# ZeldaM1/PnP-VCVE

Measured on AMD Instinct MI355X. Metric: enhanced frames/sec (1280x720, 7-frame window), higher is better.
Workload: dtype f32; 1 GPU; 1 x 7x3x720x1280 clip per GPU per step (BASELINE configs[2] shape), full BAE+CAA forward, config HR_davis_LR_128x128 generator, seeded random weights; side info per SURVEY 8(d): partition class ~ U{0,1,2} per 8x8 block (one-hot/255, none on the I frame), quarter-pel block MVs, IBBBP cadence; vsr_x4_heads=False, hip_graphs=False, deform=vos, parallelism=clip-sharded replicas x1

## Files before the change

### pnp_vcve_amd/csrc/conv_wino.hip

```cpp
#include "conv_mfma.h"
#include <cstring>
#include <type_traits>

namespace {

template <int N>
using I = std::integral_constant<int, N>;
typedef unsigned u32x4 __attribute__((ext_vector_type(4)));

constexpr int HP = 18, NPX = HP * HP;
constexpr int SLAB_B = NPX * 64;
constexpr int RING_B = 4 * 16384;
constexpr int PV_B = RING_B + 4 * SLAB_B;
constexpr int BG_B = PV_B + 256 * 48;
constexpr int DUMP_B = BG_B + 256;
constexpr int WINO_LDS = DUMP_B + 1024;
constexpr unsigned OOBW = 0xFFFFFFF0u;

__device__ __forceinline__ f32x4 mfma16(float a, float b, f32x4 c) { return __builtin_amdgcn_mfma_f32_16x16x4f32(a, b, c, 0, 0, 0); }
__device__ __forceinline__ __amdgpu_buffer_rsrc_t rsrc_of(const void* p, unsigned bytes) {
    return __builtin_amdgcn_make_buffer_rsrc(const_cast<void*>(p), 0, __builtin_amdgcn_readfirstlane((int)bytes), 0x00020000);
}
__device__ __forceinline__ f32x4 bload4(__amdgpu_buffer_rsrc_t r, unsigned voff, unsigned soff) {
    return __builtin_bit_cast(f32x4, __builtin_amdgcn_raw_buffer_load_b128(r, (int)voff, (int)soff, 0));
// ... 80 lines not shown
    if (tile >= tend) return;

    const unsigned map_bytes = (unsigned)H * (unsigned)W * 256u;
    __amdgpu_buffer_rsrc_t r_src = rsrc_of(reinterpret_cast<const char*>(MS ? a.srcs[0] : a.src) - ((long)W + 1) * 256, OOBW);
    const __amdgpu_buffer_rsrc_t r_u = rsrc_of(MS ? a.ubase : a.U, MS ? OOBW : 16u * 16384u);
    const __amdgpu_buffer_rsrc_t r_urgb = rsrc_of(MS ? a.Urgb : a.U, 4u * 4096u);
    const __amdgpu_buffer_rsrc_t r_rgb = rsrc_of(reinterpret_cast<const char*>(MS ? a.rgb : a.src) - ((long)W + 1) * 16, OOBW);
    const __amdgpu_buffer_rsrc_t r_up = rsrc_of((PAR || FO) ? a.Upar : a.U, 4u * 12288u);
    const __amdgpu_buffer_rsrc_t r_out = rsrc_of(a.out, map_bytes);
    const __amdgpu_buffer_rsrc_t r_res = rsrc_of(RES ? a.residual : a.src, RES ? map_bytes : 0u);
    const __amdgpu_buffer_rsrc_t r_par = rsrc_of(a.par, PAR ? (unsigned)(3 * a.par_plane * 4) : 0u);

    const unsigned t16 = (unsigned)t * 16u;
    const int ty = 4 * (wave >> 1) + (m >> 2), tx = 4 * (wave & 1) + (m & 3);
    const unsigned dbase0 = RING_B + ((2 * ty) * HP + tx) * 64 + kq * 16, dbase1 = dbase0 + 2 * SLAB_B;
    auto lds4 = [&](unsigned byte) -> f32x4 { return *reinterpret_cast<const f32x4*>(smem + byte); };
    auto patch = [&](auto s_c, int r, int c) -> f32x4 {
        constexpr int S = decltype(s_c)::value;
        const unsigned off = (S & 1) * SLAB_B + (r * HP + (c & 1) * 9 + (c >> 1)) * 64;
        return lds4((S < 2 ? dbase0 : dbase1) + off);
    };

    const float act_lo = a.act == 0 ? 1.f : (a.act == 1 ? 0.f : 0.1f);
    if (t < 64) *reinterpret_cast<float*>(smem + BG_B + ((t & 15) * 4 + (t >> 4)) * 4) = (a.bias ? a.bias[t] : 0.f) * (a.gamma ? a.gamma[t] : 1.f);

    f32x4 acc[16][4];
    f32x4 V[16], d0[4], d1[4], d2[4], d3[4], bf[2][4], breg[4], hreg[3], tt[4];
    unsigned hoff[6];

    auto row_tf = [&](int i) {
        f32x4 tt[4];
#pragma unroll
        for (int c = 0; c < 4; ++c) tt[c] = i == 0 ? d0[c] - d2[c] : (i == 1 ? d1[c] + d2[c] : (i == 2 ? d2[c] - d1[c] : d1[c] - d3[c]));
        V[4 * i + 0] = tt[0] - tt[2];
        V[4 * i + 1] = tt[1] + tt[2];
        V[4 * i + 2] = tt[2] - tt[1];
        V[4 * i + 3] = tt[1] - tt[3];
    };
    auto halo_offsets = [&](int tq, int y0, int x0) {
#pragma unroll
        for (int i = 0; i < 6; ++i) {
            int e = tq + 256 * i;
            e = e < NPX * 4 ? e : NPX * 4 - 1;
            const int pl = e >> 2, quad = e & 3, ry = (pl * 3641) >> 16, col = pl - ry * HP;
            const int rx = col < 9 ? 2 * col : 2 * col - 17;
            const int gy = y0 - 1 + ry, gx = x0 - 1 + rx;
            const bool inb = (unsigned)gy < (unsigned)H && (unsigned)gx < (unsigned)W;
// ... 326 lines not shown
#pragma unroll
                            for (int c = 0; c < 4; ++c)
                                tt[c] = TR == 1 ? da[c] + db[c] : da[c] - db[c];
                        }
                        if (XF && g == 17) {
#pragma unroll
                            for (int c = 0; c < 4; ++c) {
                                V[4 * TR + c] = c == 0 ? tt[0] - tt[2] : (c == 1 ? tt[1] + tt[2] : (c == 2 ? tt[2] - tt[1] : tt[1] - tt[3]));
                                asm volatile("" : "+v"(V[4 * TR + c]));
                            }
                        }
                    } else {
                        if (g >= 20 && g < 28) {
                            const int c = (g - 20) & 3;
                            if (g < 24) da[c] = patch(SR{}, RA, c);
                            else db[c] = patch(SR{}, RB, c);
                        }
#pragma unroll
                        for (int c = 0; c < 4; ++c)
                            if (g == 36) tt[c] = TR == 1 ? add4(da[c], db[c]) : sub4(da[c], db[c]);
#pragma unroll
                        for (int c = 0; c < 4; ++c)
                            if (g == 36) V[4 * TR + c] = c == 0 ? sub4(tt[0], tt[2]) : (c == 1 ? add4(tt[1], tt[2]) : (c == 2 ? sub4(tt[2], tt[1]) : sub4(tt[1], tt[3])));
                    }
                    if constexpr (FO) {
                        if (PG == 0 && g >= 14 && g < 18) wjl[g - 14] = bload4(r_up, bl, fo_so + S * 12288 + (g - 14) * 1024);
                        if (PG == 1 && g >= 2 && g < 5) *reinterpret_cast<f32x4*>(smem + PV_B + (g - 2) * 4096 + tq16) = wjl[g - 2];
                        if (PG == 1 && g == 5) wj3 = wjl[3];
                    }
                    if constexpr (PAR || FO) {
                        if ((PG == 1 || PG == 2) && (g == 11 || g == 12 || g == 13 || g == 27 || g == 28 || g == 29)) {
                            wjt[(g & 15) - 11] = lds4(PV_B + ((g & 15) - 11) * 4096 + tq16);
                        }
                        if ((PG == 1 || PG == 2) && (g == 15 || g == 31)) {
                            {
                                const int pjn = (g + 1) >> 4;
                                const float cs = ((PG == 1) == (pjn == 1)) ? foldc : -foldc;
                                const f32x4 c4 = {cs, cs, cs, cs};
#pragma unroll
                                for (int n = 0; n < 3; ++n) bf[pjn & 1][n] = __builtin_elementwise_fma(c4, wjt[n], bf[pjn & 1][n]);
                                bf[pjn & 1][3] = __builtin_elementwise_fma(c4, wj3, bf[pjn & 1][3]);
                            }
                        }
                    }
                    if (PAR && g >= 52 && g < 52 + NRING) *reinterpret_cast<f32x4*>(smem + (NC & 3) * 16384 + (g - 52) * 4096 + tq16) = breg[g - 52];
                    if (!PAR && g == 63) {
// ... 97 lines not shown
                r_src = rsrc_of(reinterpret_cast<const char*>(a.srcs[last_seg ? 0 : ks + 1]) - ((long)W + 1) * 256, OOBW);
                ref_so = last_seg ? nso : (unsigned)(ty0 * W + tx0) * 256u;
                int tqs = tq;
                asm volatile("" : "+v"(tqs));
                halo_offsets(tqs, last_seg ? nty0 : ty0, last_seg ? ntx0 : tx0);
                step(I<0>{});
                step(I<1>{});
                step(I<2>{});
                step(I<3>{});
            }
        } else {
            step(I<0>{});
            step(I<1>{});
            step(I<2>{});
            step(I<3>{});
        }
        if (a.dbg) {
            dbg_b = __builtin_amdgcn_s_memtime();
            dbg_k += dbg_b - dbg_a;
        }

        const unsigned so = (unsigned)(ty0 * W + tx0) * 256u;
        const bool partial = ty0 + 16 > H || tx0 + 16 > W;
        lds_bar();
        const int tqp = (!has_next && qtile >= 0) ? ((qquad << 6) | (tq & 63)) : tq;
        pv_request(tqp, nty0, ntx0);
        fo_request(nty0, ntx0, (!has_next && qtile >= 0) ? qquad : -1);
        auto epilogue = [&](auto partial_c) {
            constexpr bool PARTIAL = decltype(partial_c)::value;
            int te = tq;
            asm volatile("" : "+v"(te));
            const int lq = te & 63, wq = te >> 6, kqq = lq >> 4, mq = lq & 15;
            char* tr = smem + 3 * 16384 + wq * 4096;
            const unsigned wbase = (unsigned)((2 * kqq) * 8 * 64 + mq * 4);
            const unsigned rbase = (unsigned)((lq >> 2) * 64 + (lq & 3) * 16);
            unsigned go[4];
#pragma unroll
            for (int j = 0; j < 4; ++j) {
                const int row = 8 * (wq >> 1) + 2 * j + (lq >> 5), col = 8 * (wq & 1) + ((lq >> 2) & 7);
                go[j] = (unsigned)(row * W + col) * 256u + (unsigned)(lq & 3) * 16u;
                if (PARTIAL) go[j] = (ty0 + row < H && tx0 + col < W) ? go[j] : OOBW;
            }
            f32x4 rs[4];
            if (RES) {
#pragma unroll
                for (int j = 0; j < 4; ++j) rs[j] = bload4(r_res, go[j], so);
            }
#pragma unroll
            for (int n = 0; n < 4; ++n) {
                f32x4 w0[4], w1[4];
#pragma unroll
                for (int i = 0; i < 4; ++i) {
                    w0[i] = acc[i * 4 + 0][n] + acc[i * 4 + 1][n] + acc[i * 4 + 2][n];
                    w1[i] = acc[i * 4 + 1][n] - acc[i * 4 + 2][n] - acc[i * 4 + 3][n];
                }
                f32x4 y[4];
                y[0] = w0[0] + w0[1] + w0[2];
                y[1] = w1[0] + w1[1] + w1[2];
                y[2] = w0[1] - w0[2] - w0[3];
                y[3] = w1[1] - w1[2] - w1[3];
#pragma unroll
                for (int q = 0; q < 4; ++q) {
#pragma unroll
                    for (int r = 0; r < 4; ++r) *reinterpret_cast<float*>(tr + wbase + ((q >> 1) * 8 + 2 * r + (q & 1)) * 64) = y[q][r];
                }
                f32x4 o[4];
#pragma unroll
                for (int j = 0; j < 4; ++j) o[j] = *reinterpret_cast<const f32x4*>(tr + rbase + j * 1024);
#pragma unroll
                for (int j = 0; j < 4; ++j) {
                    if constexpr (!RES) o[j] = __builtin_elementwise_max(o[j], act_lo * o[j]);
                    if (RES) {
                        o[j] += rs[j];
                        if (n < 3) rs[j] = bload4(r_res, go[j], so + (n + 1) * 64);
                    }
                    bstore4(r_out, go[j], so + n * 64, o[j]);
                }
            }
        };
        if (partial) epilogue(std::true_type{});
        else epilogue(std::false_type{});
        pv_finish(tqp);
        fo_finish();
        ++dbg_n;
        if (a.dbg) dbg_e += __builtin_amdgcn_s_memtime() - dbg_b;
        if (!has_next) break;
        tile = ntile;
        ty0 = nty0;
        tx0 = ntx0;
        if constexpr (SEAM) {
            f32x4 e0[4], e1[4], e2[4];
#pragma unroll
            for (int c = 0; c < 4; ++c) {
                e0[c] = patch(I<0>{}, 0, c);
                e1[c] = patch(I<0>{}, 1, c);
                e2[c] = patch(I<0>{}, 2, c);
            }
#pragma unroll
            for (int i = 0; i < 3; ++i) {
                f32x4 tr[4];
#pragma unroll
                for (int c = 0; c < 4; ++c) tr[c] = i == 0 ? e0[c] - e2[c] : (i == 1 ? e1[c] + e2[c] : e2[c] - e1[c]);
                V[4 * i + 0] = tr[0] - tr[2];
                V[4 * i + 1] = tr[1] + tr[2];
                V[4 * i + 2] = tr[2] - tr[1];
                V[4 * i + 3] = tr[1] - tr[3];
            }
        }
    }
    if constexpr (!PAR) wait_vm<0>();
    if constexpr (!MS) {
        const int qy0 = (qtile / tiles_x) * 16 + 8 * (qquad >> 1), qx0 = (qtile % tiles_x) * 16 + 8 * (qquad & 1);
        if (qtile >= 0 && qy0 < H && qx0 < W) {
            if (a.dbg) dbg_q0 = __builtin_amdgcn_s_memtime();
            const int tyq = m >> 2, txq = m & 3;
            const unsigned wq16 = (unsigned)lane * 16u + (unsigned)wave * 1024u;
            const unsigned qb0 = RING_B + ((2 * (4 * (qquad >> 1) + tyq)) * HP + 4 * (qquad & 1) + txq) * 64 + kq * 16, qb1 = qb0 + 2 * SLAB_B;
            f32x4 Bq[2][16], Bp[2][3];
#pragma unroll
            for (int p = 0; p < 16; ++p) Bq[0][p] = bload4(r_u, wq16, (unsigned)((p >> 2) * 16384 + (p & 3) * 4096));
            if constexpr (PAR) {
#pragma unroll
                for (int j = 0; j < 3; ++j) Bp[0][j] = bload4(r_up, wq16, (unsigned)(j * 4096));
            }
            f32x4 Bf[2];
            const int foq = FO ? __builtin_amdgcn_readfirstlane(fo_next) : -1;
            const unsigned foq_so = (unsigned)(foq > 0 ? foq : 0) * 4096u;
            if constexpr (FO) Bf[0] = bload4(r_up, wq16, foq_so);
            const unsigned qo = (unsigned)((qy0 + 2 * kq) * W + qx0) * 256u + (unsigned)(wave * 16 + m) * 4u;
            float resq[16];
            if constexpr (RES) {
#pragma unroll
                for (int q = 0; q < 4; ++q)
#pragma unroll
                    for (int r = 0; r < 4; ++r) {
                        const bool inq = qy0 + 2 * kq + (q >> 1) < H && qx0 + 2 * r + (q & 1) < W;
                        resq[q * 4 + r] = bload1(r_res, inq ? qo : OOBW, (unsigned)((q >> 1) * W + 2 * r + (q & 1)) * 256u);
                    }
            }
            const float bgq = *reinterpret_cast<const float*>(smem + BG_B + (m * 4 + wave) * 4);
            if constexpr (PAR) {
#pragma unroll
                for (int n = 0; n < 1; ++n) acc[0][0] = acc[3][0] = acc[12][0] = acc[15][0] = f32x4{0.f, 0.f, 0.f, 0.f};
            }
            lds_bar();
            if (a.dbg) dbg_q1 = __builtin_amdgcn_s_memtime();
            int needq = (PAR && a.par_flags) ? __builtin_amdgcn_readfirstlane(need_next) : 7;
            const int foldq = PAR ? __builtin_amdgcn_readfirstlane(fold_next) : -1;
            const float foldcq = PAR ? __builtin_bit_cast(float, __builtin_amdgcn_readfirstlane(__builtin_bit_cast(int, foldc_next)))
                                     : (FO ? __builtin_bit_cast(float, __builtin_amdgcn_readfirstlane(__builtin_bit_cast(int, foc_next))) : 0.f);
            if (foldq >= 0) needq = 0;
#pragma unroll
            for (int s4 = 0; s4 < 4; ++s4) {
                if (s4 < 3) {
#pragma unroll
                    for (int p = 0; p < 16; ++p) Bq[(s4 + 1) & 1][p] = bload4(r_u, wq16, (unsigned)(((s4 + 1) * 4 + (p >> 2)) * 16384 + (p & 3) * 4096));
                    if constexpr (PAR) {
#pragma unroll
                        for (int j = 0; j < 3; ++j) Bp[(s4 + 1) & 1][j] = bload4(r_up, wq16, (unsigned)((s4 + 1) * 12288 + j * 4096));
                    }
                    if constexpr (FO) Bf[(s4 + 1) & 1] = bload4(r_up, wq16, (unsigned)((s4 + 1) * 12288) + foq_so);
                }
                f32x4 dq[4][4], tq4[4];
// ... 147 lines not shown
    f32x4 hv[7];
    {
#pragma unroll
        for (int i = 0; i < 7; ++i) {
            const int e = t + 256 * i, pe = e >> 4, ry = pe / 10, rx = pe - ry * 10, gy = qy0 - 1 + ry, gx = qx0 - 1 + rx;
            hv[i] = f32x4{0.f, 0.f, 0.f, 0.f};
            if (e < 1600 && (unsigned)gy < (unsigned)H && (unsigned)gx < (unsigned)W)
                hv[i] = *reinterpret_cast<const f32x4*>(a.src + ((long)gy * W + gx) * 64 + (e & 15) * 4);
        }
        if constexpr (PAR) {
#pragma unroll
            for (int j = 0; j < 3; ++j)
#pragma unroll
                for (int q = 0; q < 4; ++q) {
                    const int gy = min(qy0 + 2 * tyq + (q >> 1), H - 1), gx = min(qx0 + 2 * txq + (q & 1), W - 1);
                    praw[j][q] = a.par[(long)j * a.par_plane + (long)gy * W + gx];
                }
        }
        if constexpr (FO) {
#pragma unroll
            for (int j = 0; j < 3; ++j) praw[j][0] = a.par[(long)j * a.par_plane + (long)qy0 * W + qx0];
        }
    }
    const unsigned wq16 = (unsigned)lane * 16u + (unsigned)wave * 1024u;
    constexpr int QA = 2, QB = QA + 1;
    f32x4 Bq[QB][16], Bp[QB][FO ? 1 : 3];
#pragma unroll
    for (int s0 = 0; s0 < QA; ++s0) {
#pragma unroll
        for (int p = 0; p < 16; ++p) Bq[s0][p] = bload4(r_u, wq16, (unsigned)((s0 * 4 + (p >> 2)) * 16384 + (p & 3) * 4096));
        if constexpr (PAR) {
#pragma unroll
            for (int j = 0; j < 3; ++j) Bp[s0][j] = bload4(r_up, wq16, (unsigned)(s0 * 12288 + j * 4096));
        }
    }
    int needq = 7, foldq = -1;
    float foldcq = 0.f;
    if constexpr (FO) {
        needq = 0;
#pragma unroll
        for (int j = 2; j >= 0; --j) {
            const float uv = __builtin_bit_cast(float, __builtin_amdgcn_readfirstlane(__builtin_bit_cast(int, praw[j][0])));
            if (uv != 0.f) {
                foldq = j;
                foldcq = 0.25f * uv;
            }
        }
// ... 182 lines not shown
#pragma unroll
        for (int i = 0; i < 7; ++i) {
            const int e = t + 256 * i, pe = e >> 4, ry = pe / 10, rx = pe - ry * 10, gy = qy0 - 1 + ry, gx = qx0 - 1 + rx;
            hv[i] = f32x4{0.f, 0.f, 0.f, 0.f};
            if (e < 1600 && (unsigned)gy < (unsigned)H && (unsigned)gx < (unsigned)W)
                hv[i] = *reinterpret_cast<const f32x4*>(src + ((long)gy * W + gx) * 64 + (e & 15) * 4);
        }
    };
    auto halo_store = [&](int buf) {
#pragma unroll
        for (int i = 0; i < 7; ++i) {
            const int e = t + 256 * i;
            if (e < 1600) *reinterpret_cast<f32x4*>(smem + buf * HB + (e >> 4) * QSTR + (e & 15) * 16) = hv[i];
        }
    };
    halo_request(a.srcs[0]);
    if (t < 100) {
        const int ry = t / 10, rx = t - ry * 10, gy = qy0 - 1 + ry, gx = qx0 - 1 + rx;
        f32x4 v = {0.f, 0.f, 0.f, 0.f};
        if ((unsigned)gy < (unsigned)H && (unsigned)gx < (unsigned)W) v = *reinterpret_cast<const f32x4*>(a.rgb + ((long)gy * W + gx) * 4);
        *reinterpret_cast<f32x4*>(smem + 2 * HB + t * 16) = v;
    }
    const int tyq = m >> 2, txq = m & 3;
    const unsigned wq16 = (unsigned)lane * 16u + (unsigned)wave * 1024u;
    f32x4 Bq[2][16], Br[16];
#pragma unroll
    for (int p = 0; p < 16; ++p) Br[p] = bload4(r_urgb, (unsigned)lane * 16u, (unsigned)((p >> 2) * 4096 + (p & 3) * 1024));
#pragma unroll
    for (int p = 0; p < 16; ++p) Bq[0][p] = bload4(r_u, wq16, a.u_off[0] + (unsigned)((p >> 2) * 16384 + (p & 3) * 4096));
    halo_store(0);
    const float bgq = a.bias ? a.bias[wave * 16 + m] : 0.f;
    f32x4 acc[16], V[16];
    lds_bar();
    {
        float dr[16], tr[16], Vr[16];
#pragma unroll
        for (int r = 0; r < 4; ++r)
#pragma unroll
            for (int c = 0; c < 4; ++c) dr[r * 4 + c] = *reinterpret_cast<const float*>(smem + 2 * HB + ((2 * tyq + r) * 10 + 2 * txq + c) * 16 + kq * 4);
#pragma unroll
        for (int c = 0; c < 4; ++c) {
            tr[0 * 4 + c] = dr[0 * 4 + c] - dr[2 * 4 + c];
            tr[1 * 4 + c] = dr[1 * 4 + c] + dr[2 * 4 + c];
            tr[2 * 4 + c] = dr[2 * 4 + c] - dr[1 * 4 + c];
            tr[3 * 4 + c] = dr[1 * 4 + c] - dr[3 * 4 + c];
        }
#pragma unroll
        for (int i = 0; i < 4; ++i) {
            Vr[i * 4 + 0] = tr[i * 4 + 0] - tr[i * 4 + 2];
            Vr[i * 4 + 1] = tr[i * 4 + 1] + tr[i * 4 + 2];
            Vr[i * 4 + 2] = tr[i * 4 + 2] - tr[i * 4 + 1];
            Vr[i * 4 + 3] = tr[i * 4 + 1] - tr[i * 4 + 3];
        }
#pragma unroll
        for (int p = 0; p < 16; ++p) {
            const f32x4 c0 = p == 5 ? f32x4{bgq, bgq, bgq, bgq} : f32x4{0.f, 0.f, 0.f, 0.f};
            const float bw = wave == 0 ? Br[p][0] : (wave == 1 ? Br[p][1] : (wave == 2 ? Br[p][2] : Br[p][3]));
            acc[p] = mfma16(Vr[p], bw, c0);
        }
    }
    for (int ks = 0; ks < a.nsrc; ++ks) {
        const bool more = ks + 1 < a.nsrc;
        const int buf = ks & 1;
        if (more) halo_request(a.srcs[ks + 1]);
#pragma unroll
        for (int s4 = 0; s4 < 4; ++s4) {
            if (s4 < 3) {
#pragma unroll
                for (int p = 0; p < 16; ++p)
                    Bq[(s4 + 1) & 1][p] = bload4(r_u, wq16, a.u_off[ks] + (unsigned)(((s4 + 1) * 4 + (p >> 2)) * 16384 + (p & 3) * 4096));
            } else if (more) {
#pragma unroll
                for (int p = 0; p < 16; ++p) Bq[0][p] = bload4(r_u, wq16, a.u_off[ks + 1] + (unsigned)((p >> 2) * 16384 + (p & 3) * 4096));
            }
            f32x4 dq[4][4], tq4[4];
#pragma unroll
            for (int r = 0; r < 4; ++r)
#pragma unroll
                for (int c = 0; c < 4; ++c)
                    dq[r][c] = *reinterpret_cast<const f32x4*>(smem + buf * HB + ((2 * tyq + r) * 10 + 2 * txq + c) * QSTR + (16 * s4 + 4 * kq) * 4);
#pragma unroll
// ... 34 lines not shown
    yq[2] = w0[1] - w0[2] - w0[3];
    yq[3] = w1[1] - w1[2] - w1[3];
    const unsigned qo = (unsigned)((qy0 + 2 * kq) * W + qx0) * 256u + (unsigned)(wave * 16 + m) * 4u;
#pragma unroll
    for (int q = 0; q < 4; ++q) {
        yq[q] = __builtin_elementwise_max(yq[q], act_lo * yq[q]);
#pragma unroll
        for (int r = 0; r < 4; ++r) {
            const bool inq = qy0 + 2 * kq + (q >> 1) < H && qx0 + 2 * r + (q & 1) < W;
            bstore1(r_out, inq ? qo : OOBW, (unsigned)((q >> 1) * W + 2 * r + (q & 1)) * 256u, yq[q][r]);
        }
    }
}
#endif
#ifndef WINO_MS_TU

struct WinoImgArgs {
    const float* src[16];
    float* dst[16];
    const float* gamma;
};
__global__ __launch_bounds__(256) void wino_image_kernel(const WinoImgArgs a) {
    const int idx = blockIdx.x * 256 + threadIdx.x;
    const int ci = ((idx >> 10) & 3) * 16 + ((idx >> 6) & 3) * 4 + (idx & 3), co = ((idx >> 8) & 3) * 16 + ((idx >> 2) & 15);
    const float* s = a.src[blockIdx.y];
    float* d = a.dst[blockIdx.y];
    double g[3][3];
#pragma unroll
    for (int tap = 0; tap < 9; ++tap)
        g[tap / 3][tap % 3] = s[tap * 4096 + (((ci >> 3) * 2 + (co >> 5)) * 64 + ((ci >> 2) & 1) * 32 + (co & 31)) * 4 + (ci & 3)];
    const double gm = a.gamma ? (double)a.gamma[co] : 1.0;
    double tmp[4][3];
#pragma unroll
    for (int x = 0; x < 3; ++x) {
        tmp[0][x] = g[0][x];
        tmp[1][x] = 0.5 * (g[0][x] + g[1][x] + g[2][x]);
        tmp[2][x] = 0.5 * (g[0][x] - g[1][x] + g[2][x]);
        tmp[3][x] = g[2][x];
    }
#pragma unroll
    for (int i = 0; i < 4; ++i) {
        const double u[4] = {tmp[i][0], 0.5 * (tmp[i][0] + tmp[i][1] + tmp[i][2]), 0.5 * (tmp[i][0] - tmp[i][1] + tmp[i][2]), tmp[i][2]};
#pragma unroll
        for (int pj = 0; pj < 4; ++pj)
            d[((ci >> 4) * 4 + i) * 4096 + ((pj * 4 + (co >> 4)) * 64 + ((ci >> 2) & 3) * 16 + (co & 15)) * 4 + (ci & 3)] = (float)(u[pj] * gm);
    }
}

__global__ __launch_bounds__(256) void wino_par_image_kernel(const float* __restrict__ src, float* __restrict__ dst) {
    const int idx = blockIdx.x * 256 + threadIdx.x;
    const int br = idx >> 12, e = idx & 4095;
    const int ci = ((e >> 10) & 3) * 16 + ((e >> 6) & 3) * 4 + (e & 3), co = ((e >> 8) & 3) * 16 + ((e >> 2) & 15);
    const float v = src[br * 4096 + (((ci >> 3) * 2 + (co >> 5)) * 64 + ((ci >> 2) & 1) * 32 + (co & 31)) * 4 + (ci & 3)];
    dst[(((ci >> 4) * 3 + br) * 4 + (co >> 4)) * 256 + (((ci >> 2) & 3) * 16 + (co & 15)) * 4 + (ci & 3)] = v;
}

__global__ __launch_bounds__(256) void wino_rgb_image_kernel(const float* __restrict__ src, float* __restrict__ dst) {
    const int idx = blockIdx.x * 256 + threadIdx.x;
    const int c = idx >> 6, co = idx & 63;
    double g[3][3];
#pragma unroll
    for (int tap = 0; tap < 9; ++tap)
        g[tap / 3][tap % 3] = src[(((tap >> 1) * 2 + (co >> 5)) * 64 + (tap & 1) * 32 + (co & 31)) * 4 + c];
    double tmp[4][3];
#pragma unroll
    for (int x = 0; x < 3; ++x) {
        tmp[0][x] = g[0][x];
        tmp[1][x] = 0.5 * (g[0][x] + g[1][x] + g[2][x]);
        tmp[2][x] = 0.5 * (g[0][x] - g[1][x] + g[2][x]);
        tmp[3][x] = g[2][x];
    }
#pragma unroll
    for (int i = 0; i < 4; ++i) {
        const double u[4] = {tmp[i][0], 0.5 * (tmp[i][0] + tmp[i][1] + tmp[i][2]), 0.5 * (tmp[i][0] - tmp[i][1] + tmp[i][2]), tmp[i][2]};
#pragma unroll
        for (int pj = 0; pj < 4; ++pj) dst[i * 1024 + (pj * 64 + c * 16 + (co & 15)) * 4 + (co >> 4)] = (float)u[pj];
    }
}

#endif
}

int launch_conv3x3_wino_ms_raw(const void* wino_args, int grid, int units, int ntiles, hipStream_t stream);

#ifdef WINO_MS_TU
int launch_conv3x3_wino_ms_raw(const void* wino_args, int grid, int units, int ntiles, hipStream_t stream) {
    static PnpPerDevice once;
    int unused = 0;
    const hipError_t attr_err = once.run([](int, int&) {
        return hipFuncSetAttribute(reinterpret_cast<const void*>(conv3x3_wino_kernel<false, false, true>),
                                   hipFuncAttributeMaxDynamicSharedMemorySize, WINO_LDS);
    }, &unused);
    if (attr_err != hipSuccess) return (int)attr_err;
    const WinoArgs& w = *static_cast<const WinoArgs*>(wino_args);
    if (units) hipLaunchKernelGGL(conv3x3_wino_quad_ms_kernel, dim3(4 * ntiles), dim3(256), 0, stream, w);
    else hipLaunchKernelGGL((conv3x3_wino_kernel<false, false, true>), dim3(grid), dim3(256), WINO_LDS, stream, w);
    return (int)hipGetLastError();
}
#else
// ... 140 lines not shown
```

### pnp_vcve_amd/csrc/generator.hip

```cpp
#include <deque>
#include <string>
#include <vector>
#include <cstring>
#include <cstdlib>

#include "../../include/pnpvcve.h"
#include "../../include/pnpvcve_debug.h"
#include "abi_shared.h"
#include "conv_mfma.h"
#include "prep.h"
#include "warp.h"
#include "dcn.h"
#ifdef PNP_HOST_STUB
#include "host_stub/io_stub.h"
#endif

namespace {

struct ParamInfo {
    std::string name;
    std::vector<int64_t> shape;
    int64_t offset = 0, numel = 0;
};

// ... 508 lines not shown
    W.slots = take(hw * 64 * nslots);
    W.kw = take(hw * 64);
    W.tmp0 = take(hw * 64);
    W.tmp1 = take(hw * 64);
    if (g->cfg.vsr) {
        W.u1 = take(hw * 4 * 64);
        W.u2 = take(hw * 16 * 64);
        W.u3 = take(hw * 16 * 64);
    } else {
        W.u1 = W.u2 = W.u3 = nullptr;
    }
    if (g->cfg.deform != 0) {
        W.flow4 = take(hw * 4);
        W.om = take(hw * 448);
    } else {
        W.flow4 = W.om = nullptr;
    }
    W.parbin = g->cfg.sparse_val ? take(hw * 3 * (bounded ? 1 : t)) : nullptr;
    W.ew = take((int64_t)t * g->cfg.num_experts);
    W.gamma = take((int64_t)t * 64);
    W.mixw = take((int64_t)t * g->ndyn * IMG_WIDE);
    W.mixb = take((int64_t)t * g->ndyn * 64);
    W.mixh = g->prec != PNP_PREC_F32 ? take((int64_t)t * g->ndyn * IMG_WIDE / (g->prec == PNP_PREC_F16X3 ? 1 : 2)) : nullptr;
    W.wino = (g->prec == PNP_PREC_F32 && g->ndyn > 0) ? take((int64_t)2 * g->cfg.num_blocks * PNP_WINO_IMG_FLOATS) : nullptr;
    const bool mir = g->prec == PNP_PREC_F16 && g->cfg.deform == 0;
    W.x16 = mir ? reinterpret_cast<uint16_t*>(take(hw * 32)) : nullptr;
    W.slots16 = mir ? reinterpret_cast<uint16_t*>(take(hw * 32 * nslots)) : nullptr;
    W.parany = reinterpret_cast<int*>(take(t));
    W.parflags = reinterpret_cast<int*>(take((int64_t)t * ((w + 15) / 16) * ((h + 7) / 8)));
    W.queue = g->prec == PNP_PREC_F16X3 ? reinterpret_cast<int*>(take(16)) : nullptr;
    const bool staged = io_staged(g);
    W.lr1 = (staged && lq_format == PNP_FRAMES_U8_HWC) ? take(hw * 3) : nullptr;
    W.out1 = (staged && out_mask == PNP_OUT_U8) ? take(hw * 3 * (g->cfg.vsr ? 16 : 1)) : nullptr;
    W.bytes = off;
    return W;
}

}

int launch_fill(float* dst, float v, int n, hipStream_t stream) {
    if (n < 0 || n > 64) return PNP_ERR_BAD_ARG;
    hipLaunchKernelGGL(fill_kernel, dim3(1), dim3(64), 0, stream, dst, v, n);
    return (int)hipGetLastError();
}

int launch_small_copy(const float* src, float* dst, int n_valid, int n_total, int mode, hipStream_t stream) {
    if (n_total < 1 || mode < PNP_COPY_PAD || mode > PNP_COPY_DCN_CHANNELS) return PNP_ERR_BAD_ARG;
// ... 423 lines not shown
                a.dst_ystride = IMG_WIDE;
                rc = launch_pack_weights(a, g->ndyn, st);
                if (rc) return rc;
                rc = launch_mix_bias(flat + g->dyn_b, W.ew + (int64_t)i * E, W.mixb + (int64_t)u * g->ndyn * 64, E, 64,
                                     g->ndyn, st);
                if (rc) return rc;
                if (g->prec == PNP_PREC_F16) {
                    rc = launch_f16_image(a.dst, reinterpret_cast<uint16_t*>(W.mixh) + (int64_t)u * g->ndyn * IMG_WIDE,
                                          g->ndyn * 9, 2, st);
                    if (rc) return rc;
                }
                if (g->prec == PNP_PREC_F16X3) {
                    rc = launch_f16x3_image(a.dst, reinterpret_cast<uint16_t*>(W.mixh) + (int64_t)u * g->ndyn * IMG_WIDE * 2,
                                            g->ndyn * 9, st);
                    if (rc) return rc;
                }
            }
            uidx[i] = u;
        }
        std::vector<char> key(t);
        for (int i = 0; i < t; ++i) key[i] = (sl[i] == 73.0f) || (sl[i] == 80.0f);
        key[0] = key[t - 1] = 1;

        auto run_branch = [&](int brid, int i, int out, ConvCall in) -> int {
            const BranchPk& B = g->br[brid];
            const float* gam = (c.with_bias && c.with_se) ? W.gamma + (int64_t)i * 64 : nullptr;
            const float* parp = sparse_per_frame ? W.parbin : par_b + (int64_t)i * 3 * hw;
            const int* pflags = par_skip ? W.parflags + (int64_t)i * ((w + 15) / 16) * ((h + 7) / 8) : nullptr;
            const int* pany = (par_skip && wopt >= 1) ? W.parany + i : nullptr;
            const int u = uidx[i];
            float* slot = W.slots + (int64_t)out * fm;
            const void* x16 = (chain16 && in.nsrc > 1) ? W.x16 : nullptr;
            int r = conv(in.bias(flat + B.in_bias).act(2).units(wino_units(h, w)).to(W.tmp0).also16(const_cast<void*>(x16)));
            if (r) return r;
            const float* x = W.tmp0;
            const bool un = wino_units(h, w);
            if (wino_on && g->ndyn > 0) {
                std::vector<const float*> ws;
                std::vector<float*> wd;
                for (int k = 0; k < c.num_blocks; ++k) {
                    const BlockPk& K = B.blocks[k];
                    if (K.dyn_conv2 >= 0) { ws.push_back(W.mixw + ((int64_t)u * g->ndyn + K.dyn_conv2) * IMG_WIDE); wd.push_back(W.wino + (int64_t)(2 * k) * PNP_WINO_IMG_FLOATS); }
                    if (K.dyn_conv1 >= 0) { ws.push_back(W.mixw + ((int64_t)u * g->ndyn + K.dyn_conv1) * IMG_WIDE); wd.push_back(W.wino + (int64_t)(2 * k + 1) * PNP_WINO_IMG_FLOATS); }
                }
                for (size_t j = 0; j < ws.size(); j += 16) {
                    const int n = (int)(ws.size() - j < 16 ? ws.size() - j : 16);
                    r = launch_wino_images(ws.data() + j, wd.data() + j, n, gam, st);
                    if (r) return r;
                }
            }
            for (int k = 0; k < c.num_blocks; ++k) {
                const BlockPk& K = B.blocks[k];
                float* dst = (k == c.num_blocks - 1) ? slot : W.tmp0;
                void* dst16 = !mirrors ? nullptr : (k == c.num_blocks - 1) ? (void*)(W.slots16 + (int64_t)out * fm)
                                                                                 : (chain16 ? (void*)W.x16 : nullptr);
                const bool woqp = c.blocktype == 1;
                const float* w2 = woqp ? packed + K.conv2_img : W.mixw + ((int64_t)u * g->ndyn + K.dyn_conv2) * IMG_WIDE;
                const float* b2 = woqp ? flat + K.conv2_bias : W.mixb + ((int64_t)u * g->ndyn + K.dyn_conv2) * 64;
                const float* g2 = woqp ? nullptr : gam;
                const float* w1 = c.one_layer ? packed + K.conv1_img
                                              : W.mixw + ((int64_t)u * g->ndyn + K.dyn_conv1) * IMG_WIDE;
                const float* b1 = c.one_layer ? flat + K.conv1_bias
                                              : W.mixb + ((int64_t)u * g->ndyn + K.dyn_conv1) * 64;
                const float* g1 = c.one_layer ? nullptr : gam;
                const float* u2 = !wino_on ? nullptr : (woqp ? packed + K.conv2_wino : W.wino + (int64_t)(2 * k) * PNP_WINO_IMG_FLOATS);
                const float* u1 = !wino_on ? nullptr : (c.one_layer ? packed + K.conv1_wino : W.wino + (int64_t)(2 * k + 1) * PNP_WINO_IMG_FLOATS);
                const float* up = !wino_on ? nullptr : packed + K.w1x1_wino;
                const int o16 = f16_maps ? 1 : 0, s16 = f16_maps ? 2 : 0;
                if (c.channel_first) {
                    r = conv(ConvCall(h, w, cfg_lr).source(x, 64, w2).mirror16(x16).bias(b2).gamma(g2)
                                 .partition(packed + K.w1x1, parp, pflags).gate(pany).wino(u2, up).units(un).act(1).to(W.tmp1).f16_map(o16));
                    if (!r)
                        r = conv(ConvCall(h, w, cfg_lr).source(W.tmp1, 64, w1).bias(b1).gamma(g1).wino(u1).units(un).residual(x).to(dst)
                                     .f16_map(s16).also16(dst16));
                } else {
                    r = conv(ConvCall(h, w, cfg_lr).source(x, 64, w1).mirror16(x16).bias(b1).gamma(g1).wino(u1).units(un).act(1).to(W.tmp1)
                                 .f16_map(o16));
                    if (!r)
                        r = conv(ConvCall(h, w, cfg_lr).source(W.tmp1, 64, w2).bias(b2).gamma(g2)
                                     .partition(packed + K.w1x1, parp, pflags).gate(pany).wino(u2, up).units(un).residual(x).to(dst).f16_map(s16).also16(dst16));
                }
                if (r) return r;
                x = dst;
                x16 = chain16 ? dst16 : nullptr;
            }
            return 0;
        };

        const void* kw16 = mirrors ? (const void*)W.kw : nullptr;
        auto s16of = [&](int i) -> const void* { return mirrors ? (const void*)(W.slots16 + (int64_t)i * fm) : nullptr; };
        std::vector<Step> steps;
        int recomputed = 0;
        if (!make_schedule(g, t, key, steps, &recomputed)) return PNP_ERR_BAD_ARG;
        auto slot_of = [&](int s) { return W.slots + (int64_t)s * fm; };
        auto wi = [&](int64_t off) -> const float* { return wino_on ? packed + off : nullptr; };
        for (const Step& sp : steps) {
            const int i = sp.frame;
            const BranchPk& B = g->br[sp.sweep];
            ConvCall in(h, w, cfg_lr);
            in.source(W.lr4 + (int64_t)i * hw * 4, 4, packed + B.in_lr, wi(B.in_lr_wino));
            if (sp.key >= 0) {
                const int fp = sp.sweep == 0 ? 2 : 0;
                rc = align(slot_of(sp.key), mv_b + ((int64_t)i * 4 + fp) * hw, mv_b + ((int64_t)i * 4 + fp + 1) * hw);
                if (rc) return rc;
                if (c.with_cat && c.align_key && sp.key_frame == (sp.sweep == 0 ? i + 1 : i - 1)) {
                    in.source(W.kw, 64, packed + B.in_wide01, wi(B.in_wide01_wino)).mirror16(kw16);
                } else {
                    in.source(W.kw, 64, packed + B.in_wide[0], wi(B.in_wide_wino[0])).mirror16(kw16);
                    if (c.with_cat) in.source(slot_of(sp.nb), 64, packed + B.in_wide[1], wi(B.in_wide_wino[1])).mirror16(s16of(sp.nb));
                }
            }
            if (sp.sweep == 1)
                in.source(slot_of(sp.own), 64, packed + B.in_wide[B.n_wide - 1], wi(B.in_wide_wino[B.n_wide - 1])).mirror16(s16of(sp.own));
            if (sparse_per_frame) {
                rc = launch_par_sparse(par_in + (int64_t)i * 3 * hw, W.parbin, 1, h, w, st);
                g->prof_last = nullptr;
                if (rc) return rc;
            }
            const bool hr_in_chain = sp.sweep == 1 && !c.vsr;
            rc = chain_open(1 + 2 * c.num_blocks + (hr_in_chain ? 1 : 0));
            if (rc) return rc;
            rc = run_branch(sp.sweep, i, sp.out, in);
            if (!rc && !hr_in_chain) rc = chain_close();
            if (rc) return rc;
            if (sp.sweep == 0) continue;

            const float* feat = slot_of(sp.out);
            const float* lr_i = lr_b ? lr_b + (int64_t)i * 3 * hw : nullptr;
            float* out_i = out_b ? out_b + (int64_t)i * 3 * hw * os * os : nullptr;
            const unsigned char* lr8_i = lq8 ? lq8 + (int64_t)i * 3 * hw : nullptr;
            unsigned char* out8_i = out8 ? out8 + (int64_t)i * 3 * hw * os * os : nullptr;
            auto stage_in = [&]() -> int {
                if (!staged) return PNP_OK;
                int r = PNP_OK;
                if (lr8_i) {
                    r = launch_frames_from_rgb8(lr8_i, W.lr1, 1, h, w, st);
                    g->prof_last = nullptr;
                    lr_i = W.lr1;
                    lr8_i = nullptr;
                }
                if (out8_i && !out_i) out_i = W.out1;
                return r;
            };
            auto stage_out = [&]() -> int {
                if (!staged || !out8_i) return PNP_OK;
// ... 174 lines not shown
```

Measured before the change: 91.91 frames/s.

## Relayout Winograd weight images, register-transpose epilogue, double-buffer per-step weight transforms

Changes the packed layout of Winograd weight images so the output-channel index becomes lane-major. Each lane can then load its own bias/weight scalars directly, removing the per-wave select on the RGB path. The epilogue transposes output tiles in registers instead of bouncing them through LDS, which also drops an LDS barrier before the next-tile prefetch. The host double-buffers the dynamic weight-image buffer so the next step's weight transforms are launched before the current branch runs. This costs twice the workspace for those images, and removing the barrier risks a race if LDS reuse depended on it.

```diff
diff --git a/pnp_vcve_amd/csrc/conv_wino.hip b/pnp_vcve_amd/csrc/conv_wino.hip
--- a/pnp_vcve_amd/csrc/conv_wino.hip
+++ b/pnp_vcve_amd/csrc/conv_wino.hip
@@ -126,7 +126,7 @@
     };
 
     const float act_lo = a.act == 0 ? 1.f : (a.act == 1 ? 0.f : 0.1f);
-    if (t < 64) *reinterpret_cast<float*>(smem + BG_B + ((t & 15) * 4 + (t >> 4)) * 4) = (a.bias ? a.bias[t] : 0.f) * (a.gamma ? a.gamma[t] : 1.f);
+    if (t < 64) *reinterpret_cast<float*>(smem + BG_B + t * 4) = (a.bias ? a.bias[t] : 0.f) * (a.gamma ? a.gamma[t] : 1.f);
 
     f32x4 acc[16][4];
     f32x4 V[16], d0[4], d1[4], d2[4], d3[4], bf[2][4], breg[4], hreg[3], tt[4];
@@ -499,6 +499,10 @@
 #pragma unroll
                         for (int c = 0; c < 4; ++c)
                             if (g == 36) V[4 * TR + c] = c == 0 ? sub4(tt[0], tt[2]) : (c == 1 ? add4(tt[1], tt[2]) : (c == 2 ? sub4(tt[2], tt[1]) : sub4(tt[1], tt[3])));
+                        if (S == 3 && PG >= 1 && g == 36) {
+#pragma unroll
+                            for (int c = 0; c < 4; ++c) asm volatile("" : "+v"(V[4 * TR + c]));
+                        }
                     }
                     if constexpr (FO) {
                         if (PG == 0 && g >= 14 && g < 18) wjl[g - 14] = bload4(r_up, bl, fo_so + S * 12288 + (g - 14) * 1024);
@@ -642,7 +646,6 @@
 
         const unsigned so = (unsigned)(ty0 * W + tx0) * 256u;
         const bool partial = ty0 + 16 > H || tx0 + 16 > W;
-        lds_bar();
         const int tqp = (!has_next && qtile >= 0) ? ((qquad << 6) | (tq & 63)) : tq;
         pv_request(tqp, nty0, ntx0);
         fo_request(nty0, ntx0, (!has_next && qtile >= 0) ? qquad : -1);
@@ -651,21 +654,20 @@
             int te = tq;
             asm volatile("" : "+v"(te));
             const int lq = te & 63, wq = te >> 6, kqq = lq >> 4, mq = lq & 15;
-            char* tr = smem + 3 * 16384 + wq * 4096;
-            const unsigned wbase = (unsigned)((2 * kqq) * 8 * 64 + mq * 4);
-            const unsigned rbase = (unsigned)((lq >> 2) * 64 + (lq & 3) * 16);
-            unsigned go[4];
-#pragma unroll
-            for (int j = 0; j < 4; ++j) {
-                const int row = 8 * (wq >> 1) + 2 * j + (lq >> 5), col = 8 * (wq & 1) + ((lq >> 2) & 7);
-                go[j] = (unsigned)(row * W + col) * 256u + (unsigned)(lq & 3) * 16u;
-                if (PARTIAL) go[j] = (ty0 + row < H && tx0 + col < W) ? go[j] : OOBW;
-            }
-            f32x4 rs[4];
+            const int row = 8 * (wq >> 1) + 2 * kqq, col = 8 * (wq & 1);
+            const unsigned gb = (unsigned)(row * W + col) * 256u + (unsigned)mq * 16u;
+            auto voff = [&](int q, int r) -> unsigned {
+                const unsigned v = gb + (unsigned)(2 * r + (q & 1)) * 256u;
+                if (PARTIAL) return (ty0 + row + (q >> 1) < H && tx0 + col + 2 * r + (q & 1) < W) ? v : OOBW;
+                return v;
+            };
+            auto soff = [&](int q) -> unsigned { return so + (unsigned)((q >> 1) * W) * 256u; };
+            f32x4 rs[2][4];
             if (RES) {
 #pragma unroll
-                for (int j = 0; j < 4; ++j) rs[j] = bload4(r_res, go[j], so);
-            }
+                for (int r = 0; r < 4; ++r) rs[0][r] = bload4(r_res, voff(0, r), soff(0));
+            }
+            f32x4 o[4][4];
 #pragma unroll
             for (int n = 0; n < 4; ++n) {
                 f32x4 w0[4], w1[4];
@@ -680,21 +682,22 @@
                 y[2] = w0[1] - w0[2] - w0[3];
                 y[3] = w1[1] - w1[2] - w1[3];
 #pragma unroll
-                for (int q = 0; q < 4; ++q) {
-#pragma unroll
-                    for (int r = 0; r < 4; ++r) *reinterpret_cast<float*>(tr + wbase + ((q >> 1) * 8 + 2 * r + (q & 1)) * 64) = y[q][r];
-                }
-                f32x4 o[4];
-#pragma unroll
-                for (int j = 0; j < 4; ++j) o[j] = *reinterpret_cast<const f32x4*>(tr + rbase + j * 1024);
-#pragma unroll
-                for (int j = 0; j < 4; ++j) {
-                    if constexpr (!RES) o[j] = __builtin_elementwise_max(o[j], act_lo * o[j]);
-                    if (RES) {
-                        o[j] += rs[j];
-                        if (n < 3) rs[j] = bload4(r_res, go[j], so + (n + 1) * 64);
-                    }
-                    bstore4(r_out, go[j], so + n * 64, o[j]);
+                for (int q = 0; q < 4; ++q)
+#pragma unroll
+                    for (int r = 0; r < 4; ++r) o[q][r][n] = y[q][r];
+                __builtin_amdgcn_sched_barrier(0);
+            }
+#pragma unroll
+            for (int q = 0; q < 4; ++q) {
+                if (RES && q < 3) {
+#pragma unroll
+                    for (int r = 0; r < 4; ++r) rs[(q + 1) & 1][r] = bload4(r_res, voff(q + 1, r), soff(q + 1));
+                }
+#pragma unroll
+                for (int r = 0; r < 4; ++r) {
+                    if constexpr (!RES) o[q][r] = __builtin_elementwise_max(o[q][r], act_lo * o[q][r]);
+                    if (RES) o[q][r] += rs[q & 1][r];
+                    bstore4(r_out, voff(q, r), soff(q), o[q][r]);
                 }
             }
         };
@@ -734,7 +737,7 @@
         if (qtile >= 0 && qy0 < H && qx0 < W) {
             if (a.dbg) dbg_q0 = __builtin_amdgcn_s_memtime();
             const int tyq = m >> 2, txq = m & 3;
-            const unsigned wq16 = (unsigned)lane * 16u + (unsigned)wave * 1024u;
+            const unsigned wq16 = (unsigned)(m & 3) * 1024u + (unsigned)(kq * 16 + 4 * wave + (m >> 2)) * 16u;
             const unsigned qb0 = RING_B + ((2 * (4 * (qquad >> 1) + tyq)) * HP + 4 * (qquad & 1) + txq) * 64 + kq * 16, qb1 = qb0 + 2 * SLAB_B;
             f32x4 Bq[2][16], Bp[2][3];
 #pragma unroll
@@ -758,7 +761,7 @@
                         resq[q * 4 + r] = bload1(r_res, inq ? qo : OOBW, (unsigned)((q >> 1) * W + 2 * r + (q & 1)) * 256u);
                     }
             }
-            const float bgq = *reinterpret_cast<const float*>(smem + BG_B + (m * 4 + wave) * 4);
+            const float bgq = *reinterpret_cast<const float*>(smem + BG_B + (wave * 16 + m) * 4);
             if constexpr (PAR) {
 #pragma unroll
                 for (int n = 0; n < 1; ++n) acc[0][0] = acc[3][0] = acc[12][0] = acc[15][0] = f32x4{0.f, 0.f, 0.f, 0.f};
@@ -952,7 +955,7 @@
             for (int j = 0; j < 3; ++j) praw[j][0] = a.par[(long)j * a.par_plane + (long)qy0 * W + qx0];
         }
     }
-    const unsigned wq16 = (unsigned)lane * 16u + (unsigned)wave * 1024u;
+    const unsigned wq16 = (unsigned)(m & 3) * 1024u + (unsigned)(kq * 16 + 4 * wave + (m >> 2)) * 16u;
     constexpr int QA = 2, QB = QA + 1;
     f32x4 Bq[QB][16], Bp[QB][FO ? 1 : 3];
 #pragma unroll
@@ -1181,10 +1184,11 @@
         *reinterpret_cast<f32x4*>(smem + 2 * HB + t * 16) = v;
     }
     const int tyq = m >> 2, txq = m & 3;
-    const unsigned wq16 = (unsigned)lane * 16u + (unsigned)wave * 1024u;
-    f32x4 Bq[2][16], Br[16];
-#pragma unroll
-    for (int p = 0; p < 16; ++p) Br[p] = bload4(r_urgb, (unsigned)lane * 16u, (unsigned)((p >> 2) * 4096 + (p & 3) * 1024));
+    const unsigned wq16 = (unsigned)(m & 3) * 1024u + (unsigned)(kq * 16 + 4 * wave + (m >> 2)) * 16u;
+    f32x4 Bq[2][16];
+    float Br[16];
+#pragma unroll
+    for (int p = 0; p < 16; ++p) Br[p] = bload1(r_urgb, (unsigned)(kq * 64 + wave * 16 + m) * 4u, (unsigned)((p >> 2) * 4096 + (p & 3) * 1024));
 #pragma unroll
     for (int p = 0; p < 16; ++p) Bq[0][p] = bload4(r_u, wq16, a.u_off[0] + (unsigned)((p >> 2) * 16384 + (p & 3) * 4096));
     halo_store(0);
@@ -1214,8 +1218,7 @@
 #pragma unroll
         for (int p = 0; p < 16; ++p) {
             const f32x4 c0 = p == 5 ? f32x4{bgq, bgq, bgq, bgq} : f32x4{0.f, 0.f, 0.f, 0.f};
-            const float bw = wave == 0 ? Br[p][0] : (wave == 1 ? Br[p][1] : (wave == 2 ? Br[p][2] : Br[p][3]));
-            acc[p] = mfma16(Vr[p], bw, c0);
+            acc[p] = mfma16(Vr[p], Br[p], c0);
         }
     }
     for (int ks = 0; ks < a.nsrc; ++ks) {
@@ -1296,7 +1299,7 @@
 };
 __global__ __launch_bounds__(256) void wino_image_kernel(const WinoImgArgs a) {
     const int idx = blockIdx.x * 256 + threadIdx.x;
-    const int ci = ((idx >> 10) & 3) * 16 + ((idx >> 6) & 3) * 4 + (idx & 3), co = ((idx >> 8) & 3) * 16 + ((idx >> 2) & 15);
+    const int ci = ((idx >> 10) & 3) * 16 + ((idx >> 6) & 3) * 4 + (idx & 3), co = ((idx >> 2) & 15) * 4 + ((idx >> 8) & 3);
     const float* s = a.src[blockIdx.y];
     float* d = a.dst[blockIdx.y];
     double g[3][3];
@@ -1317,16 +1320,16 @@
         const double u[4] = {tmp[i][0], 0.5 * (tmp[i][0] + tmp[i][1] + tmp[i][2]), 0.5 * (tmp[i][0] - tmp[i][1] + tmp[i][2]), tmp[i][2]};
 #pragma unroll
         for (int pj = 0; pj < 4; ++pj)
-            d[((ci >> 4) * 4 + i) * 4096 + ((pj * 4 + (co >> 4)) * 64 + ((ci >> 2) & 3) * 16 + (co & 15)) * 4 + (ci & 3)] = (float)(u[pj] * gm);
+            d[((ci >> 4) * 4 + i) * 4096 + ((pj * 4 + (co & 3)) * 64 + ((ci >> 2) & 3) * 16 + (co >> 2)) * 4 + (ci & 3)] = (float)(u[pj] * gm);
     }
 }
 
 __global__ __launch_bounds__(256) void wino_par_image_kernel(const float* __restrict__ src, float* __restrict__ dst) {
     const int idx = blockIdx.x * 256 + threadIdx.x;
     const int br = idx >> 12, e = idx & 4095;
-    const int ci = ((e >> 10) & 3) * 16 + ((e >> 6) & 3) * 4 + (e & 3), co = ((e >> 8) & 3) * 16 + ((e >> 2) & 15);
+    const int ci = ((e >> 10) & 3) * 16 + ((e >> 6) & 3) * 4 + (e & 3), co = ((e >> 2) & 15) * 4 + ((e >> 8) & 3);
     const float v = src[br * 4096 + (((ci >> 3) * 2 + (co >> 5)) * 64 + ((ci >> 2) & 1) * 32 + (co & 31)) * 4 + (ci & 3)];
-    dst[(((ci >> 4) * 3 + br) * 4 + (co >> 4)) * 256 + (((ci >> 2) & 3) * 16 + (co & 15)) * 4 + (ci & 3)] = v;
+    dst[(((ci >> 4) * 3 + br) * 4 + (co & 3)) * 256 + (((ci >> 2) & 3) * 16 + (co >> 2)) * 4 + (ci & 3)] = v;
 }
 
 __global__ __launch_bounds__(256) void wino_rgb_image_kernel(const float* __restrict__ src, float* __restrict__ dst) {
@@ -1348,7 +1351,7 @@
     for (int i = 0; i < 4; ++i) {
         const double u[4] = {tmp[i][0], 0.5 * (tmp[i][0] + tmp[i][1] + tmp[i][2]), 0.5 * (tmp[i][0] - tmp[i][1] + tmp[i][2]), tmp[i][2]};
 #pragma unroll
-        for (int pj = 0; pj < 4; ++pj) dst[i * 1024 + (pj * 64 + c * 16 + (co & 15)) * 4 + (co >> 4)] = (float)u[pj];
+        for (int pj = 0; pj < 4; ++pj) dst[i * 1024 + (pj * 64 + c * 16) * 4 + co] = (float)u[pj];
     }
 }
 
diff --git a/pnp_vcve_amd/csrc/generator.hip b/pnp_vcve_amd/csrc/generator.hip
--- a/pnp_vcve_amd/csrc/generator.hip
+++ b/pnp_vcve_amd/csrc/generator.hip
@@ -554,7 +554,7 @@
     W.mixw = take((int64_t)t * g->ndyn * IMG_WIDE);
     W.mixb = take((int64_t)t * g->ndyn * 64);
     W.mixh = g->prec != PNP_PREC_F32 ? take((int64_t)t * g->ndyn * IMG_WIDE / (g->prec == PNP_PREC_F16X3 ? 1 : 2)) : nullptr;
-    W.wino = (g->prec == PNP_PREC_F32 && g->ndyn > 0) ? take((int64_t)2 * g->cfg.num_blocks * PNP_WINO_IMG_FLOATS) : nullptr;
+    W.wino = (g->prec == PNP_PREC_F32 && g->ndyn > 0) ? take((int64_t)2 * 2 * g->cfg.num_blocks * PNP_WINO_IMG_FLOATS) : nullptr;
     const bool mir = g->prec == PNP_PREC_F16 && g->cfg.deform == 0;
     W.x16 = mir ? reinterpret_cast<uint16_t*>(take(hw * 32)) : nullptr;
     W.slots16 = mir ? reinterpret_cast<uint16_t*>(take(hw * 32 * nslots)) : nullptr;
@@ -1024,8 +1024,31 @@
         for (int i = 0; i < t; ++i) key[i] = (sl[i] == 73.0f) || (sl[i] == 80.0f);
         key[0] = key[t - 1] = 1;
 
-        auto run_branch = [&](int brid, int i, int out, ConvCall in) -> int {
+        auto wino_buf = [&](int buf) { return W.wino + (int64_t)buf * 2 * c.num_blocks * PNP_WINO_IMG_FLOATS; };
+        auto branch_images = [&](int brid, int i, int buf) -> int {
+            if (!(wino_on && g->ndyn > 0)) return 0;
             const BranchPk& B = g->br[brid];
+            const float* gam = (c.with_bias && c.with_se) ? W.gamma + (int64_t)i * 64 : nullptr;
+            const int u = uidx[i];
+            float* wb = wino_buf(buf);
+            std::vector<const float*> ws;
+            std::vector<float*> wd;
+            for (int k = 0; k < c.num_blocks; ++k) {
+                const BlockPk& K = B.blocks[k];
+                if (K.dyn_conv2 >= 0) { ws.push_back(W.mixw + ((int64_t)u * g->ndyn + K.dyn_conv2) * IMG_WIDE); wd.push_back(wb + (int64_t)(2 * k) * PNP_WINO_IMG_FLOATS); }
+                if (K.dyn_conv1 >= 0) { ws.push_back(W.mixw + ((int64_t)u * g->ndyn + K.dyn_conv1) * IMG_WIDE); wd.push_back(wb + (int64_t)(2 * k + 1) * PNP_WINO_IMG_FLOATS); }
+            }
+            for (size_t j = 0; j < ws.size(); j += 16) {
+                const int n = (int)(ws.size() - j < 16 ? ws.size() - j : 16);
+                const int r = launch_wino_images(ws.data() + j, wd.data() + j, n, gam, st);
+                if (r) return r;
+            }
+            g->prof_last = nullptr;
+            return 0;
+        };
+        auto run_branch = [&](int brid, int i, int out, int buf, ConvCall in) -> int {
+            const BranchPk& B = g->br[brid];
+            const float* wbuf = W.wino ? wino_buf(buf) : nullptr;
             const float* gam = (c.with_bias && c.with_se) ? W.gamma + (int64_t)i * 64 : nullptr;
             const float* parp = sparse_per_frame ? W.parbin : par_b + (int64_t)i * 3 * hw;
             const int* pflags = par_skip ? W.parflags + (int64_t)i * ((w + 15) / 16) * ((h + 7) / 8) : nullptr;
@@ -1037,20 +1060,6 @@
             if (r) return r;
             const float* x = W.tmp0;
             const bool un = wino_units(h, w);
-            if (wino_on && g->ndyn > 0) {
-                std::vector<const float*> ws;
-                std::vector<float*> wd;
-                for (int k = 0; k < c.num_blocks; ++k) {
-                    const BlockPk& K = B.blocks[k];
-                    if (K.dyn_conv2 >= 0) { ws.push_back(W.mixw + ((int64_t)u * g->ndyn + K.dyn_conv2) * IMG_WIDE); wd.push_back(W.wino + (int64_t)(2 * k) * PNP_WINO_IMG_FLOATS); }
-                    if (K.dyn_conv1 >= 0) { ws.push_back(W.mixw + ((int64_t)u * g->ndyn + K.dyn_conv1) * IMG_WIDE); wd.push_back(W.wino + (int64_t)(2 * k + 1) * PNP_WINO_IMG_FLOATS); }
-                }
-                for (size_t j = 0; j < ws.size(); j += 16) {
-                    const int n = (int)(ws.size() - j < 16 ? ws.size() - j : 16);
-                    r = launch_wino_images(ws.data() + j, wd.data() + j, n, gam, st);
-                    if (r) return r;
-                }
-            }
             for (int k = 0; k < c.num_blocks; ++k) {
                 const BlockPk& K = B.blocks[k];
                 float* dst = (k == c.num_blocks - 1) ? slot : W.tmp0;
@@ -1065,8 +1074,8 @@
                 const float* b1 = c.one_layer ? flat + K.conv1_bias
                                               : W.mixb + ((int64_t)u * g->ndyn + K.dyn_conv1) * 64;
                 const float* g1 = c.one_layer ? nullptr : gam;
-                const float* u2 = !wino_on ? nullptr : (woqp ? packed + K.conv2_wino : W.wino + (int64_t)(2 * k) * PNP_WINO_IMG_FLOATS);
-                const float* u1 = !wino_on ? nullptr : (c.one_layer ? packed + K.conv1_wino : W.wino + (int64_t)(2 * k + 1) * PNP_WINO_IMG_FLOATS);
+                const float* u2 = !wino_on ? nullptr : (woqp ? packed + K.conv2_wino : wbuf + (int64_t)(2 * k) * PNP_WINO_IMG_FLOATS);
+                const float* u1 = !wino_on ? nullptr : (c.one_layer ? packed + K.conv1_wino : wbuf + (int64_t)(2 * k + 1) * PNP_WINO_IMG_FLOATS);
                 const float* up = !wino_on ? nullptr : packed + K.w1x1_wino;
                 const int o16 = f16_maps ? 1 : 0, s16 = f16_maps ? 2 : 0;
                 if (c.channel_first) {
@@ -1096,7 +1105,12 @@
         if (!make_schedule(g, t, key, steps, &recomputed)) return PNP_ERR_BAD_ARG;
         auto slot_of = [&](int s) { return W.slots + (int64_t)s * fm; };
         auto wi = [&](int64_t off) -> const float* { return wino_on ? packed + off : nullptr; };
-        for (const Step& sp : steps) {
+        if (!steps.empty()) {
+            rc = branch_images(steps[0].sweep, steps[0].frame, 0);
+            if (rc) return rc;
+        }
+        for (size_t si = 0; si < steps.size(); ++si) {
+            const Step& sp = steps[si];
             const int i = sp.frame;
             const BranchPk& B = g->br[sp.sweep];
             ConvCall in(h, w, cfg_lr);
@@ -1120,9 +1134,13 @@
                 if (rc) return rc;
             }
             const bool hr_in_chain = sp.sweep == 1 && !c.vsr;
+            if (si + 1 < steps.size()) {
+                rc = branch_images(steps[si + 1].sweep, steps[si + 1].frame, (int)((si + 1) & 1));
+                if (rc) return rc;
+            }
             rc = chain_open(1 + 2 * c.num_blocks + (hr_in_chain ? 1 : 0));
             if (rc) return rc;
-            rc = run_branch(sp.sweep, i, sp.out, in);
+            rc = run_branch(sp.sweep, i, sp.out, (int)(si & 1), in);
             if (!rc && !hr_in_chain) rc = chain_close();
             if (rc) return rc;
             if (sp.sweep == 0) continue;
```

After: 93.27 frames/s (median of 6 runs). 1.5% higher.
